# mdnunez/bayesflow_nddms

Hardware: AMD Instinct MI355X
Metric: simulated DDM trials/sec at n_trials=300 dt=0.001 (basic_ddm_dc, max_steps=4000) (higher is better)
Workload: dtype f32

## Files before the change

### bayesflow_nddms_amd/_lib.py

```python
import ctypes
import os

from .build import SO_PATH

NDDM_OK, NDDM_ERR_NULL, NDDM_ERR_SHAPE, NDDM_ERR_PARAM, NDDM_ERR_HIP, NDDM_ERR_NO_DEVICE = range(6)
GAUSS_EXACT, GAUSS_FAST, BRIDGE, GAUSS_PACKED, STATE_F64 = 0, 1, 2, 4, 8
QUANTILE_CONDITIONAL = 1
ABI_VERSION = 4

_lib = None


class NddmLibraryError(ImportError):
    pass


def _declare(L):
    c = ctypes
    fp, vp = c.c_void_p, c.c_void_p
    L.nddm_abi_version.restype = c.c_int
    L.nddm_last_error.restype = c.c_char_p
    L.nddm_device_count.argtypes = [c.POINTER(c.c_int)]
    L.nddm_set_device.argtypes = [c.c_int]
    L.nddm_summary_k.restype = c.c_int
    L.nddm_model_nparams.argtypes = [c.c_int]
    L.nddm_set_tuning.argtypes = [c.c_int] * 6
    L.nddm_set_debug_trace.argtypes = [c.c_void_p, c.c_int, c.c_int]
    L.nddm_set_ordering.argtypes = [c.c_int]
    L.nddm_debug_set_slot_limit.argtypes = [c.c_int]
    L.nddm_debug_last_launch.argtypes = [c.POINTER(c.c_int32)]
    common = [c.c_int64, c.c_int32, c.c_float, c.c_int32, c.c_uint64, c.c_uint64, c.c_uint32]
    for name in ("nddm_basic_ddm_dc_simulate", "nddm_single_trial_simulate", "nddm_single_trial_alt_simulate"):
        getattr(L, name).argtypes = [fp] + common + [fp, fp, vp]
    L.nddm_alpha_not_scaled_simulate.argtypes = [fp] + common + [c.c_float, c.c_int32, fp, fp, fp, vp]
    L.nddm_explicit_boundary_simulate.argtypes = [fp, fp] + common + [fp, fp, vp]
    L.nddm_simulratcliff.argtypes = [fp, c.c_int64, c.c_int32, c.c_uint64, c.c_uint64, c.c_uint32, c.c_float, c.c_int32, fp, fp, fp, vp]
    L.nddm_wiener_log_likelihood.argtypes = [c.c_int32, fp, c.c_int64, c.c_int64, fp, c.c_int32, c.c_uint32, fp, fp, vp]
    L.nddm_wiener_cdf.argtypes = [c.c_int32, fp, c.c_int64, c.c_int64, fp, c.c_int32, c.c_uint32, fp, fp, vp]
    L.nddm_wiener_log_likelihood_grad.argtypes = [c.c_int32, fp, c.c_int64, c.c_int64, fp, c.c_int32, c.c_uint32, fp, fp, vp]
    L.nddm_wiener_quantile.argtypes = [c.c_int32, fp, c.c_int64, c.c_int64, fp, c.c_int32, c.c_uint32, fp, vp]
    L.nddm_simulate.argtypes = [c.c_int32, fp, fp] + common + [c.c_float, c.c_int32, fp, fp, fp, vp]
    L.nddm_simulate_indirect.argtypes = [c.c_int32, fp, fp] + common[:-1] + [fp, c.c_uint32, c.c_float, c.c_int32, fp, fp, fp, vp]
    L.nddm_simulate_codes.argtypes = [c.c_int32, fp] + common[:-1] + [fp, c.c_uint32, fp, fp, fp, vp]
    L.nddm_decode_codes.argtypes = [c.c_int32, fp, fp, c.c_int64, c.c_int32, c.c_float, fp, vp]
    L.nddm_draw_prior.argtypes = [c.c_int32, c.c_int64, c.c_uint64, c.c_uint64, c.c_float, fp, vp]
    L.nddm_draw_prior_indirect.argtypes = [c.c_int32, c.c_int64, c.c_uint64, c.c_uint64, fp, c.c_float, fp, vp]
    L.nddm_graph_arena_create.argtypes = [c.POINTER(c.c_uint64)]
    L.nddm_graph_arena_bind.argtypes = [c.c_uint64, c.POINTER(c.c_uint64)]
    L.nddm_graph_arena_info.argtypes = [c.c_uint64, c.POINTER(c.c_uint64), c.POINTER(c.c_int32)]
    L.nddm_graph_arena_release.argtypes = [c.c_uint64]
    L.nddm_source_hash.restype = c.c_char_p
    L.nddm_build_info.restype = c.c_char_p
    L.nddm_debug_normals.argtypes = [fp, c.c_int64, c.c_uint32, c.c_uint32, c.c_uint32, fp, vp]
    for name in EXPORTS:
        if name not in ("nddm_last_error", "nddm_source_hash", "nddm_build_info"):
            getattr(L, name).restype = c.c_int


EXPORTS = [
    "nddm_abi_version", "nddm_last_error", "nddm_device_count", "nddm_set_device", "nddm_summary_k",
    "nddm_model_nparams", "nddm_basic_ddm_dc_simulate", "nddm_single_trial_simulate",
    "nddm_single_trial_alt_simulate", "nddm_alpha_not_scaled_simulate", "nddm_explicit_boundary_simulate",
    "nddm_simulate", "nddm_draw_prior", "nddm_debug_normals", "nddm_set_tuning", "nddm_set_debug_trace", "nddm_set_ordering",
    "nddm_release_graph_memory", "nddm_debug_set_slot_limit", "nddm_debug_last_launch",
    "nddm_simulate_indirect", "nddm_draw_prior_indirect", "nddm_source_hash", "nddm_simulate_codes", "nddm_decode_codes",
    "nddm_graph_arena_create", "nddm_graph_arena_bind", "nddm_graph_arena_info", "nddm_graph_arena_release", "nddm_build_info",
    "nddm_simulratcliff", "nddm_wiener_log_likelihood", "nddm_wiener_cdf", "nddm_wiener_quantile",
    "nddm_wiener_log_likelihood_grad",
]


def lib():
    global _lib
    if _lib is None:
        from .build import build_hip, embedded_hash, is_stale, source_hash
        override = bool(os.environ.get("NDDM_HIP_LIB"))
        if is_stale():
            try:
                build_hip()
            except Exception as e:
                why = "is missing" if not os.path.exists(SO_PATH) else \
                    f"was built from other sources (library {embedded_hash()}, tree {source_hash()})"
                raise NddmLibraryError(
                    f"{SO_PATH} {why} and could not be rebuilt ({e!r}): build it with "
                    "`python -c 'import __graft_entry__ as g; g.build()'` (hipcc --offload-arch=gfx950).  "
                    "There is no CPU fallback.") from e
        if not os.path.exists(SO_PATH):
            raise NddmLibraryError(f"{SO_PATH} does not exist (NDDM_HIP_LIB points to a missing file?).  There is no CPU fallback.")
        import torch
        try:
            L = ctypes.CDLL(SO_PATH)
        except OSError as e:
            raise NddmLibraryError(f"cannot load {SO_PATH}: {e}") from e
        missing = [name for name in EXPORTS if not hasattr(L, name)]
        if missing:
            raise NddmLibraryError(f"{SO_PATH} does not export {missing}: it is older than this binding -- rebuild it "
                                   "(`python -c 'import __graft_entry__ as g; g.build()'`)")
        _declare(L)
        if L.nddm_abi_version() != ABI_VERSION:
            raise NddmLibraryError(f"ABI mismatch: library {L.nddm_abi_version()} != binding {ABI_VERSION} "
                                   "(the random stream differs between ABI versions): rebuild the library")
        if not override and L.nddm_source_hash().decode() != source_hash():
            raise NddmLibraryError(f"{SO_PATH} reports source hash {L.nddm_source_hash().decode()} but the tree hashes to "
                                   f"{source_hash()}: rebuild the library")
        _lib = L
    return _lib


def check(rc):
    if rc == NDDM_OK:
        return
    msg = lib().nddm_last_error().decode() or f"nddm status {rc}"
    if rc in (NDDM_ERR_NULL, NDDM_ERR_SHAPE, NDDM_ERR_PARAM):
        raise ValueError(msg)
    raise RuntimeError(msg)
```

### bayesflow_nddms_amd/csrc/nddm_kernels.hip

```cpp
#include <hip/hip_runtime.h>
#include <math.h>
#include <stdint.h>
#include <stdio.h>
#include <stdlib.h>
#include <string.h>

#include <mutex>
#include <thread>

#include "../../include/nddm.h"
#include "nddm_prepass.h"
#include "nddm_ratcliff.h"
#include "nddm_rng.h"
#include "nddm_sim.h"
#include "nddm_wiener.h"
#include "nddm_wiener_cdf.h"
#include "nddm_wiener_grad.h"
#include "nddm_wiener_quantile.h"

namespace nddm {

static thread_local char g_err[512] = "";

static int fail(int code, const char *fmt, const char *detail = "")
{
    snprintf(g_err, sizeof g_err, fmt, detail);
    return code;
}

static int round_up_pow2(int v) { int p = 1; while (p < v) p <<= 1; return p; }

static int check_stream(hipStream_t st)
{
    int sdev = -1, cur = -1;
    const hipError_t e = hipStreamGetDevice(st, &sdev);
    if (e != hipSuccess) {
        (void)hipGetLastError();
        return fail(NDDM_ERR_HIP, "`stream` is not a live stream of this process's HIP runtime (destroyed, or created by another copy "
                                  "of the runtime): %s", hipGetErrorString(e));
    }
    if (hipGetDevice(&cur) == hipSuccess && st != nullptr && st != hipStreamPerThread && sdev != cur)
        return fail(NDDM_ERR_PARAM, "`stream` belongs to another device than the current one (nddm_set_device / hipSetDevice)%s");
    return NDDM_OK;
}

struct Tuning { int sets_per_chunk, ring, refill_thresh, variant, grid_waves, tile_trials, no_order; };
struct LastLaunch { int grid_waves, vkeys, ring, tile_trials, tiles_per_set, sets_per_chunk, refill_thresh, lds_bytes; };
static thread_local LastLaunch g_last = {0, 0, 0, 0, 0, 0, 0, 0};
static std::mutex g_mu;
static Tuning g_tuning = {0, 0, 0, 0, 0, 0, 0};
static unsigned long long *g_dbg = nullptr;
static int g_dbg_waves = 0, g_dbg_chunks = 0;

constexpr int MAX_DEVICES = 64;
struct DeviceInfo { int cus = 0; double clock_hz = 0.0; };
static DeviceInfo g_dev[MAX_DEVICES];

static bool device_info(int dev, DeviceInfo *out)
{
    std::lock_guard<std::mutex> lock(g_mu);
    if (g_dev[dev].cus == 0) {
        hipDeviceProp_t prop;
        if (hipGetDeviceProperties(&prop, dev) != hipSuccess) return false;
        g_dev[dev].cus = prop.multiProcessorCount > 0 ? prop.multiProcessorCount : 1;
        g_dev[dev].clock_hz = prop.clockRate > 0 ? (double)prop.clockRate * 1e3 : 2.4e9;
    }
    *out = g_dev[dev];
    return true;
}

constexpr size_t SLOT_QUEUE_BYTES = 256, SLOT_SCRATCH = 1u << 20;
constexpr int MAX_SLOTS = 256;
struct LaunchSlot {
    char *base = nullptr;
    hipEvent_t done = nullptr;
    hipStream_t stream = nullptr;
    bool busy = false;
    bool fresh = true;
};
static LaunchSlot *g_slots[MAX_DEVICES][MAX_SLOTS];
static int g_nslots[MAX_DEVICES];
static int g_slot_limit = MAX_SLOTS;

static hipError_t malloc_relaxed(void **p, size_t bytes)
{
    hipStreamCaptureMode mode = hipStreamCaptureModeRelaxed;
    (void)hipThreadExchangeStreamCaptureMode(&mode);
    const hipError_t e = hipMalloc(p, bytes);
    (void)hipThreadExchangeStreamCaptureMode(&mode);
    return e;
}

static LaunchSlot *acquire_slot_once(int dev, hipStream_t st, hipError_t *err);

static LaunchSlot *acquire_slot(int dev, hipStream_t st, hipError_t *err)
{
    for (int spin = 0; spin < (1 << 22); ++spin) {
        LaunchSlot *s = acquire_slot_once(dev, st, err);
        if (s || *err != hipErrorNotReady) return s;
        std::this_thread::yield();
    }
    return nullptr;
}

static LaunchSlot *acquire_slot_once(int dev, hipStream_t st, hipError_t *err)
// ... 180 lines not shown
#undef NDDM_ARGS
    const hipError_t e = hipGetLastError();
    if (e != hipSuccess) return fail(NDDM_ERR_HIP, "kernel launch failed: %s", hipGetErrorString(e));
    return NDDM_OK;
}

static int simulate(int model, const float *params, const float *bounds, int64_t B, int32_t n_trials, float dt,
                    int32_t max_steps, uint64_t seed, uint64_t set_offset, const uint64_t *set_offset_dev, uint32_t flags,
                    float ext_sigma, int32_t ext_mode, float *out_trials, float *out_summary, float *out_ext, void *stream,
                    uint16_t *out_codes = nullptr)
{
    g_err[0] = 0;
    int P;
    bool has_zsum;
    switch (model) {
    case NDDM_BASIC_DDM_DC: P = 5; has_zsum = false; break;
    case NDDM_SINGLE_TRIAL: P = 8; has_zsum = true; break;
    case NDDM_SINGLE_TRIAL_ALT: P = 8; has_zsum = true; break;
    case NDDM_ALPHA_NOT_SCALED: P = 6; has_zsum = false; break;
    case NDDM_EXPLICIT_BOUNDARY: P = 4; has_zsum = false; break;
    default: return fail(NDDM_ERR_PARAM, "unknown model%s");
    }
    if (B < 0 || n_trials <= 0 || max_steps < 0) return fail(NDDM_ERR_SHAPE, "B < 0, n_trials <= 0 or max_steps < 0%s");
    if (max_steps >= (1 << 30)) return fail(NDDM_ERR_SHAPE, "max_steps must be < 2^30%s");
    if (set_offset >= (1ull << 60) || set_offset + (uint64_t)B > (1ull << 60))
        return fail(NDDM_ERR_SHAPE, "set_offset + B must be <= 2^60 (the random stream is keyed by 60 bits of the set index)%s");
    if (!(dt > 0.0f) || !isfinite(dt)) return fail(NDDM_ERR_PARAM, "dt must be finite and > 0%s");
    if (flags > 15u) return fail(NDDM_ERR_PARAM, "unknown flags%s");
    const bool bridge = (flags & NDDM_BRIDGE) != 0;
    const bool packed = (flags & NDDM_GAUSS_PACKED) != 0;
    const bool f64 = (flags & NDDM_STATE_F64) != 0;
    if (f64 && ((model != NDDM_BASIC_DDM_DC && model != NDDM_SINGLE_TRIAL) || bridge || packed || out_codes))
        return fail(NDDM_ERR_PARAM, "NDDM_STATE_F64 exists for NDDM_BASIC_DDM_DC and NDDM_SINGLE_TRIAL, without NDDM_BRIDGE, NDDM_GAUSS_PACKED "
                                    "or the 2-byte wire format%s");
    if (packed && (bridge || max_steps >= 16384))
        return fail(NDDM_ERR_PARAM, "NDDM_GAUSS_PACKED needs max_steps < 2^14 and cannot be combined with NDDM_BRIDGE%s");
    if (bridge && model != NDDM_ALPHA_NOT_SCALED)
        return fail(NDDM_ERR_PARAM, "NDDM_BRIDGE is only available for NDDM_ALPHA_NOT_SCALED%s");
    if (bridge && max_steps >= (1 << 22)) return fail(NDDM_ERR_SHAPE, "max_steps must be < 2^22 with NDDM_BRIDGE%s");
    if (B == 0) return NDDM_OK;
    if (!params) return fail(NDDM_ERR_NULL, "params is NULL%s");
    if (model == NDDM_EXPLICIT_BOUNDARY && !bounds) return fail(NDDM_ERR_NULL, "bounds is NULL%s");
    if (!out_trials && !out_summary && !out_ext && !out_codes) return fail(NDDM_ERR_NULL, "no output buffer given%s");
    if (out_codes && ((model != NDDM_BASIC_DDM_DC && model != NDDM_ALPHA_NOT_SCALED) || bridge || packed || max_steps >= 16384))
        return fail(NDDM_ERR_PARAM, "the 2-byte wire format exists for NDDM_BASIC_DDM_DC and NDDM_ALPHA_NOT_SCALED without NDDM_BRIDGE "
                                    "or NDDM_GAUSS_PACKED, max_steps < 2^14%s");
    if (B * (((long long)n_trials + 511) / 512) >= (1ll << 31))
        return fail(NDDM_ERR_SHAPE, "B * ceil(n_trials / 512) must be < 2^31 per launch%s");

    if (const int rc = check_stream(reinterpret_cast<hipStream_t>(stream))) return rc;

    Tuning tun;
    unsigned long long *dbg;
    int dbg_waves, dbg_chunks;
    { std::lock_guard<std::mutex> lock(g_mu); tun = g_tuning; dbg = g_dbg; dbg_waves = g_dbg_waves; dbg_chunks = g_dbg_chunks; }
    int dev = 0;
    {
        const hipError_t e = hipGetDevice(&dev);
        if (e != hipSuccess || dev < 0 || dev >= MAX_DEVICES) return fail(NDDM_ERR_HIP, "hipGetDevice: %s", hipGetErrorString(e));
    }
    DeviceInfo di;
    if (!device_info(dev, &di)) return fail(NDDM_ERR_HIP, "hipGetDeviceProperties failed%s");
    const int simds = 4 * di.cus;
    static const int sizing_per_simd = [] { const char *e = getenv("NDDM_SIZING_WAVES_PER_SIMD"); const int v = e ? atoi(e) : 0; return v >= 1 && v <= 8 ? v : 7; }();
    const long long waves_sizing = (long long)sizing_per_simd * simds;
    const long long waves_min_chunks = (long long)(sizing_per_simd - 1) * simds;

    SimArgs A;
    memset(&A, 0, sizeof A);
    A.params = params; A.bounds = bounds; A.out_trials = out_trials; A.out_summary = out_summary; A.out_ext = out_ext;
    A.out_codes = out_codes;
    A.B = B; A.n_trials = n_trials; A.max_k = max_steps; A.dt = dt; A.sqrt_dt = sqrtf(dt);
    A.tscale = bridge ? dt * 0.00390625f : dt;
    A.k0 = (uint32_t)seed; A.k1 = (uint32_t)(seed >> 32);
    A.ext_sigma = ext_sigma; A.ext_mode = ext_mode;
    A.dbg = dbg; A.dbg_waves = dbg_waves; A.dbg_chunks = dbg_chunks;
    A.dt64 = (double)dt; A.sqrt_dt64 = sqrt((double)dt);

    const bool res16 = (flags & NDDM_BRIDGE) == 0 && max_steps < 16384;
    const size_t per_trial = res16 ? 2 : 4;
    const long long total_trials = B * (long long)n_trials;
    double est_steps = 0.25 / (double)dt;
    if (est_steps > (double)max_steps) est_steps = (double)max_steps;
    if (est_steps < 1.0) est_steps = 1.0;
    const double est_blocks = (double)total_trials * est_steps / 256.0;
    long long plan_waves = 8ll * simds;
    if (tun.grid_waves > 0) plan_waves = tun.grid_waves;
    else {
        const double cap_blocks = max_steps > 4 ? (double)max_steps * 0.25 : 1.0;
        double want = est_blocks / 300.0;
        const double crit = 3.0 * (double)simds * pow(est_blocks / cap_blocks / (2.8 * (double)simds), 0.4);
        if (crit < want) want = crit;
        if (want < (double)plan_waves) plan_waves = want < (double)simds ? simds : (long long)want;
    }
    const long long waves_for_tiles = plan_waves < waves_sizing ? plan_waves : waves_sizing;
    int tile_cap = 64;
    while (tile_cap < 512 && (long long)tile_cap * waves_for_tiles * 8 < total_trials) tile_cap <<= 1;
    int tiles = tun.tile_trials > 0 ? (n_trials + tun.tile_trials - 1) / tun.tile_trials
                                    : (n_trials <= tile_cap ? 1 : (n_trials + tile_cap - 1) / tile_cap);
    int tile_n = (n_trials + tiles - 1) / tiles;
    tiles = (n_trials + tile_n - 1) / tile_n;
    if (!tun.ring && !tun.tile_trials)
        while (tile_n > 96 && (size_t)lds_header_bytes(model) + 4u * (size_t)slot_stride_bytes(tile_n, (int)per_trial) > 5120u) {
            tiles++;
            tile_n = (n_trials + tiles - 1) / tiles;
            tiles = (n_trials + tile_n - 1) / tile_n;
        }
    const long long vB = B * (long long)tiles;
    if (vB >= (1ll << 31)) return fail(NDDM_ERR_SHAPE, "B * ceil(n_trials / 512) must be < 2^31 per launch%s");
    if ((long long)tile_n * tiles >= (1ll << 30) || n_trials >= (1 << 30))
        return fail(NDDM_ERR_SHAPE, "n_trials must be < 2^30%s");
    A.n_trials = tile_n; A.n_total = n_trials; A.tiles_per_set = tiles; A.B = vB;
    int spc = tun.sets_per_chunk;
    if (!spc) {
        spc = (900 + tile_n - 1) / tile_n;
        if (spc < 1) spc = 1;
        if (spc > 64) spc = 64;
        while (spc > 1 && vB / spc < 32 * waves_for_tiles) spc >>= 1;
        const double t_est = (double)vB * ((double)tile_n * est_steps / 256.0) * 265.0 / ((double)simds * di.clock_hz)
                             + (double)max_steps * 0.25 * 265.0 * 7.0 / di.clock_hz;
        double max_chunks = t_est * 4.0e7;
        if (max_chunks < 8.0 * (double)waves_min_chunks) max_chunks = 8.0 * (double)waves_min_chunks;
        if ((double)vB / spc > max_chunks) {
            spc = (int)((double)vB / max_chunks) + 1;
            if (spc > 64) spc = 64;
        }
    }
    const auto lds_of = [&](int r) {
        return (size_t)lds_header_bytes(model) + (size_t)r * (size_t)slot_stride_bytes(tile_n, (int)per_trial);
// ... 129 lines not shown
int nddm_model_nparams(int model)
{
    switch (model) {
    case NDDM_BASIC_DDM_DC: return 5;
    case NDDM_SINGLE_TRIAL: return 8;
    case NDDM_SINGLE_TRIAL_ALT: return 8;
    case NDDM_ALPHA_NOT_SCALED: return 6;
    case NDDM_EXPLICIT_BOUNDARY: return 4;
    }
    return -1;
}

int nddm_device_count(int *count)
{
    if (!count) return nddm::fail(NDDM_ERR_NULL, "count is NULL%s");
    const hipError_t e = hipGetDeviceCount(count);
    if (e != hipSuccess) { *count = 0; return nddm::fail(NDDM_ERR_NO_DEVICE, "hipGetDeviceCount: %s", hipGetErrorString(e)); }
    return NDDM_OK;
}

int nddm_set_device(int device)
{
    const hipError_t e = hipSetDevice(device);
    if (e != hipSuccess) return nddm::fail(NDDM_ERR_HIP, "hipSetDevice: %s", hipGetErrorString(e));
    return NDDM_OK;
}

int nddm_set_tuning(int sets_per_chunk, int ring, int refill_thresh, int variant, int grid_waves, int tile_trials)
{
    if (ring < 0 || ring == 1) return nddm::fail(NDDM_ERR_PARAM, "ring must be 0 (automatic) or >= 2%s");
    std::lock_guard<std::mutex> lock(nddm::g_mu);
    const int no_order = nddm::g_tuning.no_order;
    nddm::g_tuning = {sets_per_chunk, ring, refill_thresh, variant < 0 ? 0 : variant, grid_waves, tile_trials, no_order};
    return NDDM_OK;
}

int nddm_set_ordering(int enabled)
{
    std::lock_guard<std::mutex> lock(nddm::g_mu);
    nddm::g_tuning.no_order = enabled ? 0 : 1;
    return NDDM_OK;
}

int nddm_set_debug_trace(void *dev_u64, int wave_capacity, int chunk_capacity)
{
    if (dev_u64 && (wave_capacity < 0 || chunk_capacity < 0)) return nddm::fail(NDDM_ERR_PARAM, "negative trace capacity%s");
    std::lock_guard<std::mutex> lock(nddm::g_mu);
    nddm::g_dbg = static_cast<unsigned long long *>(dev_u64);
    nddm::g_dbg_waves = dev_u64 ? wave_capacity : 0;
    nddm::g_dbg_chunks = dev_u64 ? chunk_capacity : 0;
    return NDDM_OK;
}

int nddm_debug_last_launch(int32_t *out8)
{
    if (!out8) return nddm::fail(NDDM_ERR_NULL, "out8 is NULL%s");
    const nddm::LastLaunch &l = nddm::g_last;
    out8[0] = l.grid_waves; out8[1] = l.vkeys; out8[2] = l.ring; out8[3] = l.tile_trials; out8[4] = l.tiles_per_set;
    out8[5] = l.sets_per_chunk; out8[6] = l.refill_thresh; out8[7] = l.lds_bytes;
    return NDDM_OK;
}

int nddm_debug_set_slot_limit(int n)
{
    std::lock_guard<std::mutex> lock(nddm::g_mu);
    nddm::g_slot_limit = n < 1 ? 1 : (n > nddm::MAX_SLOTS ? nddm::MAX_SLOTS : n);
    return NDDM_OK;
}

int nddm_release_graph_memory(void)
{
    nddm::g_err[0] = 0;
    int dev = 0;
    const hipError_t e = hipGetDevice(&dev);
    if (e != hipSuccess || dev < 0 || dev >= nddm::MAX_DEVICES) return nddm::fail(NDDM_ERR_HIP, "hipGetDevice: %s", hipGetErrorString(e));
    nddm::GraphAlloc *mine = nullptr;
    {
        std::lock_guard<std::mutex> lock(nddm::g_mu);
        nddm::GraphAlloc **pp = &nddm::g_ownerless.list;
        while (*pp) {
            nddm::GraphAlloc *a = *pp;
            if (a->dev == dev) { *pp = a->next; a->next = mine; mine = a; }
            else pp = &a->next;
        }
    }
    nddm::free_list(mine);
    return NDDM_OK;
}

int nddm_graph_arena_create(uint64_t *arena)
{
    nddm::g_err[0] = 0;
    if (!arena) return nddm::fail(NDDM_ERR_NULL, "arena is NULL%s");
    std::lock_guard<std::mutex> lock(nddm::g_mu);
    nddm::GraphArena *a = new nddm::GraphArena{nddm::g_next_arena++, nullptr, nddm::g_arenas};
    nddm::g_arenas = a;
    *arena = a->id;
    return NDDM_OK;
}

int nddm_graph_arena_bind(uint64_t arena, uint64_t *previous)
{
    nddm::g_err[0] = 0;
    {
        std::lock_guard<std::mutex> lock(nddm::g_mu);
        if (!nddm::find_arena_locked(arena)) return nddm::fail(NDDM_ERR_PARAM, "unknown (or released) graph arena%s");
// ... 421 lines not shown
```

### bayesflow_nddms_amd/csrc/nddm_sim.h

```cpp
#pragma once
#include <hip/hip_runtime.h>
#include <math.h>
#include <stdint.h>

#include "../../include/nddm.h"
#include "nddm_rng.h"

namespace nddm {

constexpr int WAVE = 64;
constexpr int MAX_REJECT = 64;

typedef __attribute__((address_space(3))) uint16_t lds_u16;
typedef __attribute__((address_space(3))) uint32_t lds_u32;
typedef uint32_t u32v4 __attribute__((ext_vector_type(4)));
typedef uint32_t u32v2 __attribute__((ext_vector_type(2)));
typedef __attribute__((address_space(3))) u32v4 lds_u32v4;
typedef __attribute__((address_space(3))) u32v2 lds_u32v2;

template <int MODEL> struct ModelTraits;
template <> struct ModelTraits<NDDM_BASIC_DDM_DC>      { static constexpr int P = 5; static constexpr bool HAS_Z = false; static constexpr int TAU = 3; };
template <> struct ModelTraits<NDDM_SINGLE_TRIAL>      { static constexpr int P = 8; static constexpr bool HAS_Z = true;  static constexpr int TAU = 3; };
template <> struct ModelTraits<NDDM_SINGLE_TRIAL_ALT>  { static constexpr int P = 8; static constexpr bool HAS_Z = true;  static constexpr int TAU = 3; };
template <> struct ModelTraits<NDDM_ALPHA_NOT_SCALED>  { static constexpr int P = 6; static constexpr bool HAS_Z = false; static constexpr int TAU = 3; };
template <> struct ModelTraits<NDDM_EXPLICIT_BOUNDARY> { static constexpr int P = 4; static constexpr bool HAS_Z = true;  static constexpr int TAU = 2; };

struct SimArgs {
    const float *params;
    const float *bounds;
    float *out_trials;
    float *out_summary;
    float *out_ext;
    uint16_t *out_codes;
    long long B;
    int n_trials;
    int n_total;
    int tiles_per_set;
    unsigned long long *partials;
    const uint32_t *recs;
    int max_k;
    float dt;
    float sqrt_dt;
    float tscale;
    uint32_t k0, k1;
    int sets_per_chunk;
    int n_chunks;
    unsigned int *chunk_counter;
    int ring;
    int open_ahead;
    float ext_sigma;
    int ext_mode;
    unsigned long long *dbg;
    int dbg_waves, dbg_chunks;
    int res16;
    int refill_thresh;
    uint32_t ring_magic;
    double dt64, sqrt_dt64;
};

typedef const __attribute__((address_space(4))) SimArgs *ArgsPtr;
__device__ __forceinline__ ArgsPtr fresh_args(ArgsPtr p)
{
    asm volatile("" : "+s"(p));
    return p;
}

template <bool FAST>
struct AuxStream {
    uint32_t trial, set_lo, c3, blk, kbase;
    u32x4 x;
    __device__ __forceinline__ AuxStream(uint32_t kbase_, uint32_t set_lo_, uint32_t set_hi28, uint32_t trial_)
        : trial(trial_), set_lo(set_lo_), c3(set_hi28 | 0x10000000u), blk(0xffffffffu), kbase(kbase_) {}
    __device__ __forceinline__ void block(uint32_t b)
    {
        if (b != blk) { x = philox4x32_10_lds(set_lo, trial, c3, b, kbase); blk = b; }
    }
    __device__ __forceinline__ void first_pair(float &z0, float &z1)
    {
        block(0u);
        float r, cs, sn;
        polar_pair<FAST>(x.x, x.y, r, cs, sn);
        r *= noise_unit<FAST>(1.0f);
        z0 = r * cs; z1 = r * sn;
    }
    __device__ __forceinline__ float normal(uint32_t a)
    {
        block(a >> 2);
        const bool second = (a & 2u) != 0u;
        float r, cs, sn;
        polar_pair<FAST>(second ? x.z : x.x, second ? x.w : x.y, r, cs, sn);
        r *= noise_unit<FAST>(1.0f);
        return r * ((a & 1u) ? sn : cs);
    }
};

__device__ __forceinline__ unsigned long long wave_sum(unsigned long long v)
{
#pragma unroll
    for (int off = 32; off > 0; off >>= 1) v += __shfl_xor(v, off, WAVE);
    return v;
}
__device__ __forceinline__ int wave_sum(int v)
{
#pragma unroll
    for (int off = 32; off > 0; off >>= 1) v += __shfl_xor(v, off, WAVE);
    return v;
}

__device__ __forceinline__ int fresh_lane(int lane)
{
// ... 282 lines not shown

    const ArgsPtr Ak = (ArgsPtr)__builtin_amdgcn_kernarg_segment_ptr();
    const int lane = threadIdx.x;
    const int N = A.n_trials;

    if (lane < 10) { lds_raw[2 * lane] = A.k0 + (uint32_t)lane * 0x9E3779B9u; lds_raw[2 * lane + 1] = A.k1 + (uint32_t)lane * 0xBB67AE85u; }
    if (lane == 0) { lds_raw[28] = A.k0 + 2u * PHILOX_W0; lds_raw[29] = A.k1 + 2u * PHILOX_W1; lds_raw[30] = A.k0 + 3u * PHILOX_W0; }
    uint32_t kbase;
    {
        const uint32_t off = (uint32_t)(size_t)lds_raw;
        asm volatile("v_mov_b32 %0, %1" : "=v"(kbase) : "s"(off));
    }
    const int rshift = SMALL ? 1 : (BRIDGE ? 2 : (A.res16 ? 1 : 2));
    constexpr bool LATENT = model_has_latent(MODEL);
    const int stride = DV * 4 + (((N << rshift) + 15) & ~15);
    char *const slots = reinterpret_cast<char *>(lds_raw) + lds_header_bytes(MODEL);
    auto slot_rec = [&](int slot) { return reinterpret_cast<uint32_t *>(slots + slot * stride); };
    auto pack_slots = [&](int t) {
        const ArgsPtr R = fresh_args(Ak);
        const int s0 = ring_slot(t, R->ring, R->ring_magic);
        const int o0 = s0 * stride, o01 = (s0 + 1 == R->ring ? 0 : s0 + 1) * stride - o0;
        return (o0 & 0xffff) | (o01 << 16);
    };
    constexpr uint32_t SLOTS_OFF = lds_header_bytes(MODEL);
    constexpr uint32_t FIFO_OFF = LDS_HEADER_DWORDS * 4;
    [[maybe_unused]] int fifo_pos = 0, fifo_avail = 0;

    float w = 0.0f, h = 0.0f, mu_dt = 0.0f;
    [[maybe_unused]] double xe = 0.0, ab = 0.0, cdt = 0.0, sdc = 0.0;
    int k = 0;
    [[maybe_unused]] float ta = 0.0f, tb = 0.0f;
    [[maybe_unused]] uint32_t jraw = 0;
    uint32_t res_addr = 0;
    [[maybe_unused]] int tile = 0;
    bool invalid = false;
    unsigned long long has_m = 0ull, act_m = 0ull;
    constexpr int MAX_BLOCKS = 16;
    [[maybe_unused]] int cap_k = -1;
    PathCtr pc = {0u, 0u, 0u, 0u, 0u};
    [[maybe_unused]] PathKeys pkeys;
    if constexpr (VKEYS) pkeys.init(A.k0, A.k1);

    int tile_open = 0;
    int flushed = 0;
    int next_tile = 0, next_trial = 0;
    int to_retire = N;
    int chunk_set = 0, chunk_left = 0;
    int slot_pack = pack_slots(0);
    int dirty = 1;
    unsigned long long dbg_cnt = 0;
    unsigned long long *dbg_stamp = reinterpret_cast<unsigned long long *>(lds_raw + 20);
    if (lane == 0) {
        dbg_stamp[3] = 0;
        lds_raw[31] = blockIdx.x;
        if (Ak->dbg) { dbg_stamp[0] = __builtin_amdgcn_s_memtime(); dbg_stamp[1] = __builtin_amdgcn_s_memrealtime(); }
    }

    uint32_t pre = 0u;

    auto open_tiles = [&]() {
        const ArgsPtr R = fresh_args(Ak);
        while (tile_open < flushed + R->ring && tile_open <= next_tile + R->open_ahead) {
            const bool have_pre = chunk_left > 0;
            if (chunk_left <= 0) {
                if (chunk_left < 0) break;
                unsigned int c = 0;
                if (fresh_lane(lane) == 0) c = atomicAdd(R->chunk_counter, 1u);
                c = __builtin_amdgcn_readfirstlane(c);
                if (c >= (unsigned int)R->n_chunks) {
                    chunk_left = -1;
                    if (fresh_lane(lane) == 0 && R->dbg) dbg_stamp[3] = __builtin_amdgcn_s_memrealtime();
                    break;
                }
                if (fresh_lane(lane) == 0 && R->dbg && c < (unsigned int)R->dbg_chunks)
                    R->dbg[8ll * R->dbg_waves + c] = __builtin_amdgcn_s_memrealtime();
                chunk_set = (int)c * R->sets_per_chunk;
                const long long left = R->B - (long long)chunk_set;
                chunk_left = (int)(left < R->sets_per_chunk ? left : R->sets_per_chunk);
            }
            const int slot = ring_slot(tile_open, R->ring, R->ring_magic);
            const int TPS = R->tiles_per_set;
            const int prow = TPS == 1 ? chunk_set : chunk_set / TPS;
            const int qt = chunk_set - prow * TPS;
            uint32_t rec = pre;
            if (!have_pre) rec = fresh_lane(lane) < REC ? R->recs[(long long)prow * REC + lane] : 0u;
            if (chunk_left > 1) {
                const int nrow = TPS == 1 ? chunk_set + 1 : (chunk_set + 1) / TPS;
                if (nrow != prow) pre = fresh_lane(lane) < REC ? R->recs[(long long)nrow * REC + lane] : 0u;
                else pre = rec;
            }
            const int sic = __builtin_amdgcn_readlane((int)rec, R_SET);
            const int vset = sic * TPS + qt;
            uint32_t *d = slot_rec(slot);
            if (lane < REC) d[lane] = rec;
            const uint32_t s_lo = (uint32_t)__builtin_amdgcn_readlane((int)rec, R_GLO);
            const uint32_t s_hi = (uint32_t)__builtin_amdgcn_readlane((int)rec, R_GHI);
            if (lane == 0) {
                d[D_VSET] = (uint32_t)vset;
                if constexpr (MODEL == NDDM_SINGLE_TRIAL || MODEL == NDDM_SINGLE_TRIAL_ALT) { d[D_ZSUM] = 0u; d[D_ZSUM + 1] = 0u; d[D_ZSUM + 2] = 0u; d[D_ZSUM + 3] = 0u; }
                PathSet ps;
                ps.init(s_lo, s_hi, R->k0, R->k1);
                d[D_CA] = ps.cA; d[D_CB] = ps.cB; d[D_HP1K] = ps.hP1k; d[D_X1] = ps.X1;
                d[D_SETLO] = s_lo;
                d[D_C3] = s_hi;
                d[D_TBASE] = (uint32_t)(qt * N);
            }
// ... 124 lines not shown
                if constexpr (F64) {
                    double beta64;
                    if constexpr (MODEL == NDDM_BASIC_DDM_DC) { ab = (double)a2; beta64 = (double)a3; }
                    else {
                        ab = (double)a3 + (double)a2 * (double)latent;
                        if (!(ab > 0.0)) ab = __builtin_fabs(ab);
                        beta64 = (double)__uint_as_float(rw[D_B + 2]);
                    }
                    xe = ab * beta64;
                    cdt = (double)a0 * H->dt64;
                    sdc = H->sqrt_dt64 * (double)a1;
                    if constexpr (FAST) sdc *= 1.1774100225154747;
                } else if constexpr (MODEL == NDDM_BASIC_DDM_DC) {
                    mu_dt = a0; h = a2; w = a3;
                } else if constexpr (MODEL == NDDM_SINGLE_TRIAL) {
                    const float a = latent;
                    const float hv = 0.5f * a;
                    mu_dt = a0;
                    h = hv * a1;
                    w = (a * __uint_as_float(rw[D_B + 2]) - hv) * a1;
                } else if constexpr (MODEL == NDDM_SINGLE_TRIAL_ALT) {
                    const float sig_c = latent;
                    const float inv_t = 1.0f / noise_unit<FAST>(H->sqrt_dt * sig_c);
                    const float hv = 0.5f * a1;
                    mu_dt = (a0 * H->dt) * inv_t;
                    h = hv * inv_t;
                    w = (a1 * a2 - hv) * inv_t;
                } else if constexpr (MODEL == NDDM_ALPHA_NOT_SCALED) {
                    mu_dt = latent;
                    h = a2; w = a3;
                } else if constexpr (MODEL == NDDM_EXPLICIT_BOUNDARY) {
                    const float a = trial < (uint32_t)H->n_total ? H->bounds[(long long)d2.x * H->n_total + trial] : 1.0f;
                    invalid = !(a >= 0.0f);
                    const float hv = 0.5f * a;
                    mu_dt = a0;
                    h = invalid ? 0.0f : hv * a1;
                    w = (a * a2 - hv) * a1;
                }
                const uint4 kq = *reinterpret_cast<const uint4 *>(lds_raw + 28);
                pc.init(d1.x, d1.y, d1.z, d1.w, trial, kq.x, kq.y, kq.z);
                k = 0;
                if constexpr (BRIDGE) { ta = h - __builtin_fabsf(w); tb = ta; jraw = 0u; }
            }
            if constexpr (LATENT) { const int n_ok = (int)__popcll(ok_mask); fifo_pos += n_ok; fifo_avail -= n_ok; }
            if constexpr (BRIDGE) act_m = __builtin_amdgcn_ballot_w64(ta > 0.0f) & __builtin_amdgcn_ballot_w64(k < A.max_k) & has_m;
            else if constexpr (F64) act_m = __builtin_amdgcn_ballot_w64(xe > 0.0) & __builtin_amdgcn_ballot_w64(xe < ab) & __builtin_amdgcn_ballot_w64(k < A.max_k) & has_m;
            else if constexpr (CAP4 && !PACKED) {
                const int max_k = fresh_args(Ak)->max_k;
                act_m = max_k > 0 ? __builtin_amdgcn_ballot_w64(in_range(w, h)) & has_m : 0ull;
                const int near_from = A.refill_thresh < WAVE ? max_k - 4 * MAX_BLOCKS : (int)0x80000000;
                cap_k = (__builtin_amdgcn_ballot_w64(k >= near_from) & has_m) ? max_k : -1;
            }
            else act_m = __builtin_amdgcn_ballot_w64(in_range(w, h)) & __builtin_amdgcn_ballot_w64(k < A.max_k) & has_m;
        }
        const int it_limit = A.refill_thresh < WAVE ? MAX_BLOCKS - 1 : 0x7fffffff;
        const int occupied = (int)__popcll(has_m);
        const int leave_at = occupied < A.refill_thresh ? occupied : A.refill_thresh;
        int it = 0;
        for (;; ++it) {
            if constexpr (BRIDGE) {
                const uint32_t blk = (uint32_t)k;
                const u32x4 u4 = philox4x32_10_path(blk | 0x80000000u, pc, kbase);
                unsigned long long &live = act_m;
#pragma unroll
                for (int half = 0; half < 2; ++half) {
                    const u32x4 rb = philox4x32_10_path(blk + 4u * (uint32_t)half, pc, kbase);
                    float r0, r1, c0, c1, c2, c3;
                    polar_pair<FAST, true>(rb.x, rb.y, r0, c0, c1);
                    polar_pair<FAST, true>(rb.z, rb.w, r1, c2, c3);
                    const uint32_t ua = half ? u4.z : u4.x, ub = half ? u4.w : u4.y;
                    if constexpr (FAST && CAP4) {
                        float m, uf;
#define NDDM_BSTEP(R, T, D0, D1, CVT, KLIT) "v_fmac_f32 %[w], %[" R "], %[" T "]\n\tv_add_f32 %[w], %[mu], %[w]\n\tv_sub_f32 %[" D1 "], %[h], |%[w]|\n\t" \
    "v_mul_f32 %[m], %[" D0 "], %[" D1 "]\n\tv_fmaak_f32 %[m], -4.0, %[m], " KLIT "\n\tv_exp_f32 %[m], %[m]\n\t" CVT                        \
    "v_cmpx_ge_f32_e64 vcc, %[uf], %[m]\n\tv_add_u32 %[k], 1, %[k]\n\t"
#define NDDM_U32(W) "v_cvt_f32_u32 %[uf], %[" W "]\n\t"
#define NDDM_U16(W) "v_and_b32 %[uf], 0xffff, %[" W "]\n\tv_cvt_f32_u32 %[uf], %[uf]\n\t"
                        asm volatile("s_mov_b64 exec, %[lm]\n\t"
                                     "v_mov_b32 %[jr], %[ua]\n\t"
                                     NDDM_BSTEP("r0", "c0", "ta", "tb", NDDM_U32("ua"), "0x42000001")
                                     NDDM_BSTEP("r0", "c1", "tb", "ta", NDDM_U16("ua"), "0x41800000")
                                     "v_mov_b32 %[jr], %[ub]\n\t"
                                     NDDM_BSTEP("r1", "c2", "ta", "tb", NDDM_U32("ub"), "0x42000001")
                                     NDDM_BSTEP("r1", "c3", "tb", "ta", NDDM_U16("ub"), "0x41800000")
                                     "s_nop 1\n\ts_mov_b64 %[lm], exec\n\ts_mov_b64 exec, -1"
                                     : [w] "+v"(w), [k] "+v"(k), [ta] "+v"(ta), [tb] "+v"(tb), [jr] "+v"(jraw), [lm] "+s"(live), [m] "=&v"(m),
                                       [uf] "=&v"(uf)
                                     : [mu] "v"(mu_dt), [h] "v"(h), [r0] "v"(r0), [r1] "v"(r1), [c0] "v"(c0), [c1] "v"(c1),
                                       [c2] "v"(c2), [c3] "v"(c3), [ua] "v"(ua), [ub] "v"(ub)
                                     : "vcc");
#undef NDDM_BSTEP
#undef NDDM_U32
#undef NDDM_U16
                    } else {
                        bool active = __builtin_amdgcn_inverse_ballot_w64(live);
                        const float rr4[4] = {r0, r0, r1, r1}, tt4[4] = {c0, c1, c2, c3};
#pragma unroll
                        for (int j = 0; j < 4; ++j) {
                            if (active) {
                                asm volatile("" ::: "memory");
                                const uint32_t word = j < 2 ? ua : ub;
                                const float w1 = __builtin_fmaf(rr4[j], tt4[j], w) + mu_dt;
                                const float t1 = h - __builtin_fabsf(w1);
                                const float m = ((j & 1) ? tb : ta) * t1;
                                if (j & 1) ta = t1; else tb = t1;
                                if ((j & 1) == 0) jraw = word;
// ... 67 lines not shown
                             NDDM_STEP("r0", "t1", "")      "s_xor_b64 %[am], %[am], vcc\n\t"
                             NDDM_STEP("r1", "t2", NDDM_K2) "s_xor_b64 %[am], %[am], vcc\n\t"
                             NDDM_STEP("r1", "t3", "")      "s_andn2_b64 %[am], %[am], vcc\n\t"
                             "s_cbranch_scc0 1f\n\t"
                             "s_mov_b64 exec, %[am]\n\t"
                             "v_subrev_u32 %[k], 1, %[k]\n"
                             "1:\n\t"
                             "s_mov_b64 %[am], vcc\n\t"
                             "s_mov_b64 exec, -1\n\t"
                             "s_cmp_lt_i32 %[ck], 0\n\t"
                             "s_cbranch_scc1 2f\n\t"
                             "v_cmp_gt_i32 vcc, %[ck], %[k]\n\t"
                             "s_and_b64 %[am], %[am], vcc\n"
                             "2:"
                             : [w] "+v"(w), [k] "+v"(k), [am] "+s"(act_m)
                             : [ck] "s"(cap_k), [mu] "v"(mu_dt), [h] "v"(h), [r0] "v"(rr[0]), [r1] "v"(rr[2]),
                               [t0] "v"(tt[0]), [t1] "v"(tt[1]), [t2] "v"(tt[2]), [t3] "v"(tt[3])
                             : "vcc", "scc");
#undef NDDM_STEP
#undef NDDM_K2
                if ((int)__popcll(has_m & ~act_m) >= leave_at) break;
                if (it >= it_limit) break;
                continue;
            }
#pragma unroll
            for (int j = 0; j < NS; ++j) {
                if (active) {
                    asm volatile("" ::: "memory");
                    w = __builtin_fmaf(rr[j], tt[j], w) + mu_dt;
                    k++;
                    if (j < NS - 1) {
                        if constexpr (CAP4) active = in_range(w, h);
                        else active = in_range(w, h) && (k < A.max_k);
                    }
                }
            }
            act_m = __builtin_amdgcn_ballot_w64(in_range(w, h)) & __builtin_amdgcn_ballot_w64(k < A.max_k) & has_m;
            if ((int)__popcll(has_m & ~act_m) >= leave_at) break;
            if (it >= it_limit) break;
        }
        dbg_cnt += (1ull << 32) | (unsigned long long)(uint32_t)(it + 1);
    }
    if (lane == 0) {
        unsigned int *const q = fresh_args(Ak)->chunk_counter;
        const unsigned int left = atomicAdd(q + 1, 1u);
        if (left == gridDim.x - 1u) { atomicExch(q, 0u); atomicExch(q + 1, 0u); }
    }
    unsigned long long *const dbg = fresh_args(Ak)->dbg;
    if (dbg && lane == 0) {
        const unsigned long long t_end = __builtin_amdgcn_s_memrealtime(), c_end = __builtin_amdgcn_s_memtime();
        const uint32_t wg = lds_raw[31];
        if (wg < (uint32_t)fresh_args(Ak)->dbg_waves) {
            unsigned long long *const r = dbg + 8ull * wg;
            r[0] = dbg_cnt & 0xffffffffull; r[1] = dbg_cnt >> 32;
            r[2] = c_end - dbg_stamp[0]; r[3] = t_end - dbg_stamp[1];
            r[4] = dbg_stamp[1]; r[5] = dbg_stamp[3]; r[6] = t_end; r[7] = 1ull;
        }
    }
}

}
```

### bayesflow_nddms_amd/engine.py

```python
import math
import os
import threading

import numpy as np

from . import _lib

BASIC_DDM_DC, SINGLE_TRIAL, SINGLE_TRIAL_ALT, ALPHA_NOT_SCALED, EXPLICIT_BOUNDARY = range(5)
SUMMARY_K = 10
SUMMARY_COLS = ("n_upper", "n_lower", "n_missing", "mean_rt", "var_rt", "mean_rt_upper", "var_rt_upper",
                "mean_z", "var_z", "choice_mean")
NPARAMS = {BASIC_DDM_DC: 5, SINGLE_TRIAL: 8, SINGLE_TRIAL_ALT: 8, ALPHA_NOT_SCALED: 6, EXPLICIT_BOUNDARY: 4}
_POSITIVE_COLS = {BASIC_DDM_DC: (1, 4), SINGLE_TRIAL: (5,), SINGLE_TRIAL_ALT: (1,), ALPHA_NOT_SCALED: (1, 5),
                  EXPLICIT_BOUNDARY: (3,)}

DEFAULT_FAST = True


def _torch():
    import torch
    return torch


def require_device():
# ... 474 lines not shown
            n = hi - lo
            tr = bufs[b]["trials"][:n] if want_trials else None
            sm = bufs[b]["summary"][:n] if want_summary else None
            r = simulate(model, params[lo:hi], n_trials, set_offset=_u64(set_offset + lo),
                         bounds=None if bounds is None else bounds[lo:hi], out_trials=tr, out_summary=sm, **common)
            ev = torch.cuda.Event()
            ev.record(cur)
            side.wait_event(ev)
            with torch.cuda.stream(side):
                for k in ("trials", "summary", "ext"):
                    if host[k] is not None:
                        host[k][lo:hi].copy_(r[k], non_blocking=True)
                        r[k].record_stream(side)
                copied[b] = torch.cuda.Event()
                copied[b].record(side)
        side.synchronize()
    for k, h in host.items():
        if h is not None:
            res[k] = h.numpy()
    return res


def debug_normals(counters, k0, k1, fast=False):
    torch = require_device()
    c = torch.as_tensor(np.asarray(counters, dtype=np.uint32).view(np.int32)).cuda().contiguous()
    n = c.shape[0]
    out = torch.empty((n, 4), dtype=torch.float32, device=c.device)
    rc = _lib.lib().nddm_debug_normals(c.data_ptr(), n, int(k0), int(k1), 1 if fast else 0, out.data_ptr(),
                                       torch.cuda.current_stream().cuda_stream)
    _lib.check(rc)
    return out.cpu().numpy()


class debug_trace:

    def __init__(self, waves=16384, chunks=0, device=None):
        torch = require_device()
        self.waves, self.chunks = int(waves), int(chunks)
        dev = _device(device)
        self.buf = torch.zeros(8 * self.waves + self.chunks, dtype=torch.int64, device=dev)

    def __enter__(self):
        _lib.check(_lib.lib().nddm_set_debug_trace(self.buf.data_ptr(), self.waves, self.chunks))
        return self

    def __exit__(self, *exc):
        require_device().cuda.synchronize()
        _lib.lib().nddm_set_debug_trace(None, 0, 0)
        return False

    def read(self):
        d = self.buf.cpu().numpy()
        rec = d[:8 * self.waves].reshape(self.waves, 8)
        rec = rec[rec[:, 7] == 1]
        pulls = d[8 * self.waves:]
        return {"blocks": float(rec[:, 0].sum()), "refills": float(rec[:, 1].sum()), "cycles": float(rec[:, 2].sum()),
                "ticks": float(rec[:, 3].sum()), "waves": int(rec.shape[0]), "records": rec, "pulls": pulls[pulls > 0]}


def release_graph_memory():
    _lib.check(_lib.lib().nddm_release_graph_memory())


class GraphArena:

    def __init__(self):
        import ctypes
        h = ctypes.c_uint64(0)
        _lib.check(_lib.lib().nddm_graph_arena_create(ctypes.byref(h)))
        self.handle = int(h.value)

    def bound(self):
        return _ArenaBinding(self)

    def info(self):
        import ctypes
        b, n = ctypes.c_uint64(0), ctypes.c_int32(0)
        _lib.check(_lib.lib().nddm_graph_arena_info(self.handle, ctypes.byref(b), ctypes.byref(n)))
        return {"bytes": int(b.value), "allocations": int(n.value)}

    @property
    def released(self):
        return self.handle == 0

    def release(self):
        if self.handle:
            h, self.handle = self.handle, 0
            _lib.check(_lib.lib().nddm_graph_arena_release(h))


class _ArenaBinding:
    def __init__(self, arena):
        self.arena, self.prev = arena, None

    def __enter__(self):
        import ctypes
        if self.arena.released:
            raise RuntimeError("this GraphArena has been released")
        prev = ctypes.c_uint64(0)
        _lib.check(_lib.lib().nddm_graph_arena_bind(self.arena.handle, ctypes.byref(prev)))
        self.prev = int(prev.value)
        return self.arena

    def __exit__(self, *exc):
        L = _lib.lib()
        if L.nddm_graph_arena_bind(self.prev, None) != 0:
            L.nddm_graph_arena_bind(0, None)
        return False


# ... 22 lines not shown
```

### include/nddm.h

```cpp
#ifndef NDDM_H
#define NDDM_H

#include <stdint.h>

#ifdef __cplusplus
extern "C" {
#endif

#define NDDM_ABI_VERSION 4
#define NDDM_SUMMARY_K 10

enum nddm_summary_col {
    NDDM_S_N_UPPER = 0,
    NDDM_S_N_LOWER = 1,
    NDDM_S_N_MISSING = 2,
    NDDM_S_MEAN_RT = 3,
    NDDM_S_VAR_RT = 4,
    NDDM_S_MEAN_RT_UPPER = 5,
    NDDM_S_VAR_RT_UPPER = 6,
    NDDM_S_MEAN_Z = 7,
    NDDM_S_VAR_Z = 8,
    NDDM_S_CHOICE_MEAN = 9
};

enum nddm_model {
    NDDM_BASIC_DDM_DC = 0,
    NDDM_SINGLE_TRIAL = 1,
    NDDM_SINGLE_TRIAL_ALT = 2,
    NDDM_ALPHA_NOT_SCALED = 3,
    NDDM_EXPLICIT_BOUNDARY = 4
};

enum nddm_status {
    NDDM_OK = 0,
    NDDM_ERR_NULL = 1,
    NDDM_ERR_SHAPE = 2,
    NDDM_ERR_PARAM = 3,
    NDDM_ERR_HIP = 4,
    NDDM_ERR_NO_DEVICE = 5
};

enum nddm_flags {
    NDDM_GAUSS_EXACT = 0,
    NDDM_GAUSS_FAST = 1,
    NDDM_GAUSS_PACKED = 4,
    NDDM_STATE_F64 = 8,
    NDDM_BRIDGE = 2
};

int nddm_abi_version(void);
const char *nddm_last_error(void);
int nddm_device_count(int *count);
int nddm_set_device(int device);
int nddm_summary_k(void);
int nddm_model_nparams(int model);
int nddm_graph_arena_create(uint64_t *arena);
int nddm_graph_arena_bind(uint64_t arena, uint64_t *previous );
int nddm_graph_arena_info(uint64_t arena, uint64_t *bytes , int32_t *n_allocations );
int nddm_graph_arena_release(uint64_t arena);
int nddm_release_graph_memory(void);
int nddm_debug_set_slot_limit(int n);
int nddm_debug_last_launch(int32_t *out8);
int nddm_set_tuning(int sets_per_chunk, int ring, int refill_thresh, int variant, int grid_waves, int tile_trials);
int nddm_set_ordering(int enabled);
int nddm_set_debug_trace(void *dev_u64, int wave_capacity, int chunk_capacity);


int nddm_basic_ddm_dc_simulate(const float *params, int64_t B, int32_t n_trials, float dt, int32_t max_steps,
                               uint64_t seed, uint64_t set_offset, uint32_t flags, float *out_trials,
                               float *out_summary, void *stream);

int nddm_single_trial_simulate(const float *params, int64_t B, int32_t n_trials, float dt, int32_t max_steps,
                               uint64_t seed, uint64_t set_offset, uint32_t flags, float *out_trials,
                               float *out_summary, void *stream);

int nddm_single_trial_alt_simulate(const float *params, int64_t B, int32_t n_trials, float dt, int32_t max_steps,
                                   uint64_t seed, uint64_t set_offset, uint32_t flags, float *out_trials,
                                   float *out_summary, void *stream);

int nddm_alpha_not_scaled_simulate(const float *params, int64_t B, int32_t n_trials, float dt, int32_t max_steps,
                                   uint64_t seed, uint64_t set_offset, uint32_t flags, float ext_sigma,
                                   int32_t ext_mode, float *out_trials, float *out_summary, float *out_extdata,
                                   void *stream);

int nddm_simulratcliff(const float *params, int64_t B, int32_t n_trials, uint64_t seed, uint64_t set_offset, uint32_t flags,
                       float ext_sigma, int32_t ext_mode, float *out_trials, float *out_summary, float *out_extdata, void *stream);

int nddm_wiener_log_likelihood(int32_t model, const float *params, int64_t R, int64_t draws_per_dataset, const float *data,
                               int32_t n_trials, uint32_t flags, float *out_trial_logp ,
                               double *out_loglik , void *stream);

int nddm_wiener_log_likelihood_grad(int32_t model, const float *params, int64_t R, int64_t draws_per_dataset, const float *data,
                                    int32_t n_trials, uint32_t flags , double *out_loglik ,
                                    double *out_grad , void *stream);

int nddm_wiener_cdf(int32_t model, const float *params, int64_t R, int64_t draws_per_dataset, const float *data, int32_t n_trials,
                    uint32_t flags , float *out_cdf ,
                    float *out_p_upper , void *stream);

#define NDDM_QUANTILE_CONDITIONAL 1u
int nddm_wiener_quantile(int32_t model, const float *params, int64_t R, int64_t draws_per_dataset,
                         const float *probs , int32_t n,
                         uint32_t flags , float *out_q , void *stream);

int nddm_explicit_boundary_simulate(const float *params, const float *bounds, int64_t B, int32_t n_trials,
                                    float dt, int32_t max_steps, uint64_t seed, uint64_t set_offset,
                                    uint32_t flags, float *out_trials, float *out_summary, void *stream);

int nddm_simulate(int32_t model, const float *params, const float *bounds, int64_t B, int32_t n_trials, float dt,
                  int32_t max_steps, uint64_t seed, uint64_t set_offset, uint32_t flags, float ext_sigma, int32_t ext_mode,
                  float *out_trials, float *out_summary, float *out_extdata, void *stream);

int nddm_simulate_indirect(int32_t model, const float *params, const float *bounds, int64_t B, int32_t n_trials, float dt,
                           int32_t max_steps, uint64_t seed, uint64_t set_offset, const uint64_t *set_offset_dev, uint32_t flags,
                           float ext_sigma, int32_t ext_mode, float *out_trials, float *out_summary, float *out_extdata,
                           void *stream);

int nddm_simulate_codes(int32_t model, const float *params, int64_t B, int32_t n_trials, float dt, int32_t max_steps,
// ... 23 lines not shown
```

Baseline: 9.593 billion.

## Add wave-cooperative tail mode that advances a few straggler trials using all lanes

When a wave has no more work to pull and only a few lanes (by default two) still have trials running, the new path walks those trials one at a time. All 64 lanes generate Philox normals for the same trial at once, and the steps are then applied serially through readlane broadcasts, four steps per lane. This aims to cut the idle-lane cost of long-running tail trials, which otherwise use one lane per step. The price is heavy readlane/scalar serial work per step, plus a new runtime knob and extra debug counters.

```diff
diff --git a/bayesflow_nddms_amd/_lib.py b/bayesflow_nddms_amd/_lib.py
--- a/bayesflow_nddms_amd/_lib.py
+++ b/bayesflow_nddms_amd/_lib.py
@@ -27,6 +27,7 @@
     L.nddm_set_tuning.argtypes = [c.c_int] * 6
     L.nddm_set_debug_trace.argtypes = [c.c_void_p, c.c_int, c.c_int]
     L.nddm_set_ordering.argtypes = [c.c_int]
+    L.nddm_set_tail_mode.argtypes = [c.c_int]
     L.nddm_debug_set_slot_limit.argtypes = [c.c_int]
     L.nddm_debug_last_launch.argtypes = [c.POINTER(c.c_int32)]
     common = [c.c_int64, c.c_int32, c.c_float, c.c_int32, c.c_uint64, c.c_uint64, c.c_uint32]
@@ -66,7 +67,7 @@
     "nddm_simulate_indirect", "nddm_draw_prior_indirect", "nddm_source_hash", "nddm_simulate_codes", "nddm_decode_codes",
     "nddm_graph_arena_create", "nddm_graph_arena_bind", "nddm_graph_arena_info", "nddm_graph_arena_release", "nddm_build_info",
     "nddm_simulratcliff", "nddm_wiener_log_likelihood", "nddm_wiener_cdf", "nddm_wiener_quantile",
-    "nddm_wiener_log_likelihood_grad",
+    "nddm_wiener_log_likelihood_grad", "nddm_set_tail_mode",
 ]
 
 
diff --git a/bayesflow_nddms_amd/csrc/nddm_kernels.hip b/bayesflow_nddms_amd/csrc/nddm_kernels.hip
--- a/bayesflow_nddms_amd/csrc/nddm_kernels.hip
+++ b/bayesflow_nddms_amd/csrc/nddm_kernels.hip
@@ -51,6 +51,8 @@
 static Tuning g_tuning = {0, 0, 0, 0, 0, 0, 0};
 static unsigned long long *g_dbg = nullptr;
 static int g_dbg_waves = 0, g_dbg_chunks = 0;
+static int g_tail_mode = 0;
+constexpr int TAIL_LANES_AUTO = 2;
 
 constexpr int MAX_DEVICES = 64;
 struct DeviceInfo { int cus = 0; double clock_hz = 0.0; };
@@ -337,8 +339,8 @@
 
     Tuning tun;
     unsigned long long *dbg;
-    int dbg_waves, dbg_chunks;
-    { std::lock_guard<std::mutex> lock(g_mu); tun = g_tuning; dbg = g_dbg; dbg_waves = g_dbg_waves; dbg_chunks = g_dbg_chunks; }
+    int dbg_waves, dbg_chunks, tail_mode;
+    { std::lock_guard<std::mutex> lock(g_mu); tun = g_tuning; dbg = g_dbg; dbg_waves = g_dbg_waves; dbg_chunks = g_dbg_chunks; tail_mode = g_tail_mode; }
     int dev = 0;
     {
         const hipError_t e = hipGetDevice(&dev);
@@ -360,6 +362,7 @@
     A.k0 = (uint32_t)seed; A.k1 = (uint32_t)(seed >> 32);
     A.ext_sigma = ext_sigma; A.ext_mode = ext_mode;
     A.dbg = dbg; A.dbg_waves = dbg_waves; A.dbg_chunks = dbg_chunks;
+    A.tail_lanes = tail_mode < 0 ? 0 : (tail_mode == 0 ? TAIL_LANES_AUTO : tail_mode);
     A.dt64 = (double)dt; A.sqrt_dt64 = sqrt((double)dt);
 
     const bool res16 = (flags & NDDM_BRIDGE) == 0 && max_steps < 16384;
@@ -595,6 +598,14 @@
     return NDDM_OK;
 }
 
+int nddm_set_tail_mode(int lanes)
+{
+    if (lanes < -1 || lanes > 64) return nddm::fail(NDDM_ERR_PARAM, "tail mode must be -1 (off), 0 (automatic) or 1..64 lanes%s");
+    std::lock_guard<std::mutex> lock(nddm::g_mu);
+    nddm::g_tail_mode = lanes;
+    return NDDM_OK;
+}
+
 int nddm_debug_last_launch(int32_t *out8)
 {
     if (!out8) return nddm::fail(NDDM_ERR_NULL, "out8 is NULL%s");
diff --git a/bayesflow_nddms_amd/csrc/nddm_sim.h b/bayesflow_nddms_amd/csrc/nddm_sim.h
--- a/bayesflow_nddms_amd/csrc/nddm_sim.h
+++ b/bayesflow_nddms_amd/csrc/nddm_sim.h
@@ -56,6 +56,7 @@
     int refill_thresh;
     uint32_t ring_magic;
     double dt64, sqrt_dt64;
+    int tail_lanes;
 };
 
 typedef const __attribute__((address_space(4))) SimArgs *ArgsPtr;
@@ -444,6 +445,7 @@
     unsigned long long *dbg_stamp = reinterpret_cast<unsigned long long *>(lds_raw + 20);
     if (lane == 0) {
         dbg_stamp[3] = 0;
+        dbg_stamp[2] = 0;
         lds_raw[31] = blockIdx.x;
         if (Ak->dbg) { dbg_stamp[0] = __builtin_amdgcn_s_memtime(); dbg_stamp[1] = __builtin_amdgcn_s_memrealtime(); }
     }
@@ -674,6 +676,56 @@
                 cap_k = (__builtin_amdgcn_ballot_w64(k >= near_from) & has_m) ? max_k : -1;
             }
             else act_m = __builtin_amdgcn_ballot_w64(in_range(w, h)) & __builtin_amdgcn_ballot_w64(k < A.max_k) & has_m;
+        }
+        if constexpr (!BRIDGE && !F64 && !PACKED) {
+            if (chunk_left < 0 && next_tile >= tile_open && act_m != 0ull &&
+                (int)__popcll(act_m) <= fresh_args(Ak)->tail_lanes) {
+                auto bcast_u = [](uint32_t v, int l) { return (uint32_t)__builtin_amdgcn_readlane((int)v, l); };
+                auto bcast_f = [](float v, int l) { return __uint_as_float((uint32_t)__builtin_amdgcn_readlane((int)__float_as_uint(v), l)); };
+                auto in_vgpr = [](float v) { asm volatile("v_mov_b32 %0, %0" : "+v"(v)); return v; };
+                auto all = [](bool c) { return __builtin_amdgcn_ballot_w64(c) != 0ull; };
+                do {
+                    const int L = (int)__builtin_ctzll(act_m);
+                    const int max_k = fresh_args(Ak)->max_k;
+                    const PathCtr pcb = {bcast_u(pc.cA, L), bcast_u(pc.cB, L), bcast_u(pc.cC, L), bcast_u(pc.cD, L), bcast_u(pc.cE, L)};
+                    const float hb = in_vgpr(bcast_f(h, L)), mub = in_vgpr(bcast_f(mu_dt, L));
+                    float wb = in_vgpr(bcast_f(w, L));
+                    int kb = __builtin_amdgcn_readlane(k, L);
+                    bool running = true;
+                    do {
+                        const uint32_t draw = (uint32_t)kb + 4u * (uint32_t)fresh_lane(lane);
+                        u32x4 rb;
+                        if constexpr (VKEYS) rb = philox4x32_10_path(draw, pcb, pkeys);
+                        else rb = philox4x32_10_path(draw, pcb, kbase);
+                        float r0, r1, t0, t1, t2, t3;
+                        polar_pair<FAST, true>(rb.x, rb.y, r0, t0, t1);
+                        polar_pair<FAST, true>(rb.z, rb.w, r1, t2, t3);
+#pragma nounroll
+                        for (int j = 0; j < WAVE; ++j) {
+                            const float a0 = bcast_f(r0, j), a1 = bcast_f(r1, j);
+                            const float w1 = __builtin_fmaf(a0, bcast_f(t0, j), wb) + mub;
+                            const float w2 = __builtin_fmaf(a0, bcast_f(t1, j), w1) + mub;
+                            const float w3 = __builtin_fmaf(a1, bcast_f(t2, j), w2) + mub;
+                            const float w4 = __builtin_fmaf(a1, bcast_f(t3, j), w3) + mub;
+                            const float m3 = __builtin_fmaxf(__builtin_fmaxf(__builtin_fabsf(w1), __builtin_fabsf(w2)), __builtin_fabsf(w3));
+                            if (all(m3 < hb) && all(in_range(w4, hb)) && kb + 4 < max_k) { wb = w4; kb += 4; continue; }
+                            if (!all(in_range(w1, hb)) || kb + 1 >= max_k) { wb = w1; kb += 1; }
+                            else if (!all(in_range(w2, hb)) || kb + 2 >= max_k) { wb = w2; kb += 2; }
+                            else if (!all(in_range(w3, hb)) || kb + 3 >= max_k) { wb = w3; kb += 3; }
+                            else { wb = w4; kb += 4; }
+                            running = false;
+                            break;
+                        }
+                    } while (running);
+                    const uint32_t n_steps = (uint32_t)(kb - __builtin_amdgcn_readlane(k, L)), n_batches = (n_steps + 255u) >> 8;
+                    dbg_cnt += (unsigned long long)n_batches;
+                    if (fresh_lane(lane) == 0) { lds_raw[24] += n_batches; lds_raw[25] += n_steps; }
+                    if (fresh_lane(lane) == L) { w = wb; k = kb; }
+                    act_m &= act_m - 1ull;
+                } while (act_m != 0ull);
+                dbg_cnt += 1ull << 32;
+                continue;
+            }
         }
         const int it_limit = A.refill_thresh < WAVE ? MAX_BLOCKS - 1 : 0x7fffffff;
         const int occupied = (int)__popcll(has_m);
@@ -847,7 +899,8 @@
         const uint32_t wg = lds_raw[31];
         if (wg < (uint32_t)fresh_args(Ak)->dbg_waves) {
             unsigned long long *const r = dbg + 8ull * wg;
-            r[0] = dbg_cnt & 0xffffffffull; r[1] = dbg_cnt >> 32;
+            r[0] = (dbg_cnt & 0xffffffffull) | ((unsigned long long)lds_raw[24] << 32);
+            r[1] = (dbg_cnt >> 32) | ((unsigned long long)lds_raw[25] << 32);
             r[2] = c_end - dbg_stamp[0]; r[3] = t_end - dbg_stamp[1];
             r[4] = dbg_stamp[1]; r[5] = dbg_stamp[3]; r[6] = t_end; r[7] = 1ull;
         }
diff --git a/bayesflow_nddms_amd/engine.py b/bayesflow_nddms_amd/engine.py
--- a/bayesflow_nddms_amd/engine.py
+++ b/bayesflow_nddms_amd/engine.py
@@ -550,10 +550,13 @@
     def read(self):
         d = self.buf.cpu().numpy()
         rec = d[:8 * self.waves].reshape(self.waves, 8)
-        rec = rec[rec[:, 7] == 1]
+        rec = rec[rec[:, 7] == 1].copy()
+        tail = rec[:, :2] >> 32
+        rec[:, :2] &= 0xffffffff
         pulls = d[8 * self.waves:]
         return {"blocks": float(rec[:, 0].sum()), "refills": float(rec[:, 1].sum()), "cycles": float(rec[:, 2].sum()),
-                "ticks": float(rec[:, 3].sum()), "waves": int(rec.shape[0]), "records": rec, "pulls": pulls[pulls > 0]}
+                "ticks": float(rec[:, 3].sum()), "waves": int(rec.shape[0]), "records": rec, "pulls": pulls[pulls > 0],
+                "tail_batches": float(tail[:, 0].sum()), "tail_steps": float(tail[:, 1].sum()), "tail_records": tail}
 
 
 def release_graph_memory():
diff --git a/include/nddm.h b/include/nddm.h
--- a/include/nddm.h
+++ b/include/nddm.h
@@ -64,6 +64,7 @@
 int nddm_set_tuning(int sets_per_chunk, int ring, int refill_thresh, int variant, int grid_waves, int tile_trials);
 int nddm_set_ordering(int enabled);
 int nddm_set_debug_trace(void *dev_u64, int wave_capacity, int chunk_capacity);
+int nddm_set_tail_mode(int lanes);
 
 
 int nddm_basic_ddm_dc_simulate(const float *params, int64_t B, int32_t n_trials, float dt, int32_t max_steps,
```

Result: no change. 9.603 billion (median of 6 runs) (+0.1%).
